# revdotcom/reverb

Measured on AMD Instinct MI355X. Metric: RTFx (audio-sec/wall-sec) Reverb-ASR attention_rescoring, higher is better.
Workload: dtype bf16

## Files before the change

### reverb_amd/csrc/fbank.hip

```cpp
#include <algorithm>
#include <cmath>
#include <vector>

#include "../../include/rvb.h"
#include "common.h"
#include "kernels.h"

namespace rvb {

static constexpr int WIN = 400, SHIFT = 160, NFFT = 512, NBIN = 257, NMEL = 80;

__device__ __forceinline__ void fbank_frame(const float (&x)[7], bool live, int lane, float* re, float* im, float* out,
                                            const FbankTables& t) {
  float sum = 0.f;
#pragma unroll
  for (int i = 0; i < 7; ++i) sum += x[i];
  const float mean = wave_sum(sum) / (float)WIN;
#pragma unroll
  for (int i = 0; i < 7; ++i) {
    const int j = lane + 64 * i;
    if (j < WIN) im[j] = x[i] - mean;
  }
  __syncthreads();
  float y[8];
#pragma unroll
  for (int i = 0; i < 8; ++i) {
    const int j = lane + 64 * i;
    float v = 0.f;
    if (j < WIN) {
      const float cur = im[j];
      const float prev = im[j > 0 ? j - 1 : 0];
      v = (cur - 0.97f * prev) * t.window[j];
    }
    y[i] = v;
  }
  __syncthreads();
#pragma unroll
  for (int i = 0; i < 8; ++i) {
    const int j = lane + 64 * i;
    re[__brev((unsigned)j) >> 23] = y[i];
    im[j] = 0.f;
  }
  __syncthreads();
#pragma unroll 1
  for (int s = 0; s < 9; ++s) {
    const int half = 1 << s;
#pragma unroll
    for (int q = 0; q < 4; ++q) {
      const int b = lane + 64 * q;
      const int j = b & (half - 1);
      const int i0 = ((b >> s) << (s + 1)) + j;
      const int i1 = i0 + half;
      const int tw = j << (8 - s);
      const float wr = t.twiddle[2 * tw], wi = t.twiddle[2 * tw + 1];
      const float ar = re[i0], ai = im[i0], br = re[i1], bi = im[i1];
      const float tr = wr * br - wi * bi;
      const float ti = wr * bi + wi * br;
      re[i0] = ar + tr; im[i0] = ai + ti;
      re[i1] = ar - tr; im[i1] = ai - ti;
    }
    __syncthreads();
  }
  float pw[5];
#pragma unroll
  for (int i = 0; i < 5; ++i) {
    const int j = lane + 64 * i;
    pw[i] = (j < NBIN) ? re[j] * re[j] + im[j] * im[j] : 0.f;
  }
  __syncthreads();
#pragma unroll
  for (int i = 0; i < 5; ++i) {
    const int j = lane + 64 * i;
    if (j < NBIN) re[j] = pw[i];
  }
  __syncthreads();
  if (live) {
#pragma unroll
    for (int i = 0; i < 2; ++i) {
      const int m = lane + 64 * i;
      if (m < NMEL) {
        const int lo = t.mel_lo[m], hi = t.mel_hi[m];
        const float* wrow = t.mel_w + (size_t)m * NBIN;
        float acc = 0.f;
        for (int b = lo; b < hi; ++b) acc += re[b] * wrow[b];
        out[m] = logf(fmaxf(acc, 1.1920928955078125e-07f));
      }
    }
  }
}

template <typename In>
__device__ __forceinline__ void fbank_load(const In* __restrict__ src, bool live, int lane, float (&x)[7]) {
#pragma unroll
  for (int i = 0; i < 7; ++i) {
    const int j = lane + 64 * i;
    x[i] = (live && j < WIN) ? (float)src[j] : 0.f;
  }
}

template <typename In>
__global__ __launch_bounds__(256) void fbank_kernel(const In* __restrict__ pcm, int64_t n_frames,
                                                    float* __restrict__ feats, FbankTables t) {
  __shared__ float s_re[4][NFFT];
  __shared__ float s_im[4][NFFT];
  const int lane = threadIdx.x & 63;
  const int w = threadIdx.x >> 6;
  const int64_t frame = (int64_t)blockIdx.x * 4 + w;
  const bool live = frame < n_frames;
  float x[7];
  fbank_load(pcm + frame * SHIFT, live, lane, x);
  fbank_frame(x, live, lane, s_re[w], s_im[w], feats + frame * NMEL, t);
}

__global__ __launch_bounds__(256) void fbank_batch_kernel(const int16_t* __restrict__ pcm, const float* __restrict__ wave,
                                                          const int64_t* __restrict__ frame0, const FbankRec* __restrict__ rec,
                                                          int n_rec, float* __restrict__ feats, FbankTables t) {
  __shared__ float s_re[4][NFFT];
  __shared__ float s_im[4][NFFT];
  const int lane = threadIdx.x & 63;
  const int w = __builtin_amdgcn_readfirstlane(threadIdx.x >> 6);
  const int64_t frame = (int64_t)blockIdx.x * 4 + w;
  const bool live = frame < frame0[n_rec];
  float x[7];
  float* out = feats;
  if (live) {
    int lo = 0, hi = n_rec;
    while (hi - lo > 1) {
      const int mid = (lo + hi) >> 1;
      if (frame0[mid] <= frame) lo = mid; else hi = mid;
    }
    const FbankRec r = rec[lo];
    const int64_t local = frame - frame0[lo];
    out = feats + (r.row0 + local) * NMEL;
    if (r.is_float) fbank_load(wave + r.src + local * SHIFT, true, lane, x);
    else fbank_load(pcm + r.src + local * SHIFT, true, lane, x);
  } else {
#pragma unroll
    for (int i = 0; i < 7; ++i) x[i] = 0.f;
  }
  fbank_frame(x, live, lane, s_re[w], s_im[w], out, t);
}

int fbank(hipStream_t s, const int16_t* pcm, int64_t n_frames, float* feats, const FbankTables& t) {
  if (n_frames <= 0) return OK;
  hipLaunchKernelGGL(fbank_kernel<int16_t>, dim3(cdiv(n_frames, 4)), dim3(256), 0, s, pcm, n_frames, feats, t);
  RVB_HIP_CHECK(hipGetLastError());
  return OK;
}

int fbank_f32(hipStream_t s, const float* wave, int64_t n_frames, float* feats, const FbankTables& t) {
  if (n_frames <= 0) return OK;
  hipLaunchKernelGGL(fbank_kernel<float>, dim3(cdiv(n_frames, 4)), dim3(256), 0, s, wave, n_frames, feats, t);
  RVB_HIP_CHECK(hipGetLastError());
  return OK;
}

int fbank_batch(hipStream_t s, const int16_t* pcm, const float* wave, const int64_t* frame0, const FbankRec* rec, int n_rec,
                int64_t total_frames, float* feats, int64_t n_rows, const FbankTables& t) {
  if (n_rows > 0) RVB_HIP_CHECK(hipMemsetAsync(feats, 0, (size_t)n_rows * NMEL * 4, s));
  if (total_frames <= 0 || n_rec <= 0) return OK;
  hipLaunchKernelGGL(fbank_batch_kernel, dim3(cdiv(total_frames, 4)), dim3(256), 0, s, pcm, wave, frame0, rec, n_rec, feats, t);
  RVB_HIP_CHECK(hipGetLastError());
  return OK;
}

template <typename In>
__global__ __launch_bounds__(256) void resample_kernel(const In* __restrict__ pcm, int64_t n_in, const float* __restrict__ ker,
                                                       int orig, int new_, int width, int K, float* __restrict__ out,
                                                       int64_t n_out) {
  const int64_t n = (int64_t)blockIdx.x * 256 + threadIdx.x;
  if (n >= n_out) return;
  const int64_t j = n / new_;
  const int p = (int)(n - j * new_);
  const int64_t base = j * orig - width;
  const float* kr = ker + (size_t)p * K;
  float acc = 0.f;
  for (int k = 0; k < K; ++k) {
    const int64_t i = base + k;
    if (i >= 0 && i < n_in) acc = fmaf(kr[k], (float)pcm[i], acc);
  }
  out[n] = acc;
}
int resample(hipStream_t s, const int16_t* pcm, int64_t n_in, const float* ker, int orig, int new_, int width, int K, float* out,
             int64_t n_out) {
  if (n_out <= 0) return OK;
  hipLaunchKernelGGL(resample_kernel<int16_t>, dim3(cdiv(n_out, 256)), dim3(256), 0, s, pcm, n_in, ker, orig, new_, width, K, out, n_out);
  RVB_HIP_CHECK(hipGetLastError());
  return OK;
}

int resample_f32(hipStream_t s, const float* pcm, int64_t n_in, const float* ker, int orig, int new_, int width, int K, float* out,
             int64_t n_out) {
  if (n_out <= 0) return OK;
  hipLaunchKernelGGL(resample_kernel<float>, dim3(cdiv(n_out, 256)), dim3(256), 0, s, pcm, n_in, ker, orig, new_, width, K, out, n_out);
  RVB_HIP_CHECK(hipGetLastError());
  return OK;
}

void resample_taps(int sample_rate, int target, std::vector<float>* ker, int* orig_out, int* new_out, int* width_out, int* K_out) {
  int a = sample_rate, b = target;
  while (b) { const int t = a % b; a = b; b = t; }
  const int orig = sample_rate / a, nw = target / a;
  const double lpw = 6.0, rolloff = 0.99;
  const double base_freq = std::min(orig, nw) * rolloff;
  const int width = (int)std::ceil(lpw * orig / base_freq);
  const int K = 2 * width + orig;
  ker->assign((size_t)nw * K, 0.f);
  const double PI = 3.14159265358979323846;
  for (int p = 0; p < nw; ++p)
    for (int k = 0; k < K; ++k) {
      double t = (-(double)p / nw + (double)(k - width) / orig) * base_freq;
      t = std::max(-lpw, std::min(lpw, t));
      const double c = std::cos(t * PI / lpw / 2.0);
      const double window = c * c;
      t *= PI;
      const double sinc = t == 0.0 ? 1.0 : std::sin(t) / t;
      (*ker)[(size_t)p * K + k] = (float)(sinc * window * (base_freq / orig));
    }
  *orig_out = orig; *new_out = nw; *width_out = width; *K_out = K;
}

struct FbankAny { int win, shift, nmel; };
__global__ __launch_bounds__(256) void fbank_any_kernel(const float* __restrict__ wave, int64_t n_frames, float* __restrict__ feats,
                                                        FbankTables t, FbankAny g) {
  __shared__ float s_re[4][NFFT];
  __shared__ float s_im[4][NFFT];
  const int lane = threadIdx.x & 63;
  const int w = threadIdx.x >> 6;
  const int64_t frame = (int64_t)blockIdx.x * 4 + w;
  const bool live = frame < n_frames;
  float* re = s_re[w];
  float* im = s_im[w];
  float x[8];
  float sum = 0.f;
  const float* src = wave + frame * g.shift;
#pragma unroll
  for (int i = 0; i < 8; ++i) {
    const int j = lane + 64 * i;
    x[i] = (live && j < g.win) ? src[j] : 0.f;
    sum += x[i];
  }
  const float mean = wave_sum(sum) / (float)g.win;
#pragma unroll
  for (int i = 0; i < 8; ++i) {
    const int j = lane + 64 * i;
    if (j < g.win) im[j] = x[i] - mean;
  }
  __syncthreads();
  float y[8];
#pragma unroll
  for (int i = 0; i < 8; ++i) {
    const int j = lane + 64 * i;
    float v = 0.f;
    if (j < g.win) v = (im[j] - 0.97f * im[j > 0 ? j - 1 : 0]) * t.window[j];
    y[i] = v;
  }
  __syncthreads();
#pragma unroll
  for (int i = 0; i < 8; ++i) {
    const int j = lane + 64 * i;
    re[__brev((unsigned)j) >> 23] = y[i];
    im[j] = 0.f;
  }
  __syncthreads();
#pragma unroll 1
  for (int s = 0; s < 9; ++s) {
    const int half = 1 << s;
#pragma unroll
    for (int q = 0; q < 4; ++q) {
      const int b = lane + 64 * q;
      const int j = b & (half - 1);
      const int i0 = ((b >> s) << (s + 1)) + j;
      const int i1 = i0 + half;
      const int tw = j << (8 - s);
      const float wr = t.twiddle[2 * tw], wi = t.twiddle[2 * tw + 1];
      const float ar = re[i0], ai = im[i0], br = re[i1], bi = im[i1];
      const float tr = wr * br - wi * bi;
      const float ti = wr * bi + wi * br;
      re[i0] = ar + tr; im[i0] = ai + ti;
      re[i1] = ar - tr; im[i1] = ai - ti;
    }
    __syncthreads();
  }
  float pw[5];
#pragma unroll
  for (int i = 0; i < 5; ++i) {
    const int j = lane + 64 * i;
    pw[i] = (j < NBIN) ? re[j] * re[j] + im[j] * im[j] : 0.f;
  }
  __syncthreads();
#pragma unroll
  for (int i = 0; i < 5; ++i) {
    const int j = lane + 64 * i;
    if (j < NBIN) re[j] = pw[i];
  }
  __syncthreads();
  if (live) {
#pragma unroll
    for (int i = 0; i < 2; ++i) {
      const int m = lane + 64 * i;
      if (m < g.nmel) {
        const int lo = t.mel_lo[m], hi = t.mel_hi[m];
        const float* wrow = t.mel_w + (size_t)m * NBIN;
        float acc = 0.f;
        for (int b = lo; b < hi; ++b) acc += re[b] * wrow[b];
        feats[frame * g.nmel + m] = logf(fmaxf(acc, 1.1920928955078125e-07f));
      }
    }
  }
}

void fbank_host_tables(int win, int nmel, std::vector<float>* window, std::vector<float>* tw, std::vector<float>* melw,
                       std::vector<int32_t>* lo, std::vector<int32_t>* hi) {
  const double PI = 3.14159265358979323846;
  window->resize(win); tw->resize(2 * 256); melw->assign((size_t)nmel * NBIN, 0.f);
  lo->assign(nmel, NBIN); hi->assign(nmel, 0);
  for (int i = 0; i < win; ++i) (*window)[i] = (float)std::pow(0.5 - 0.5 * std::cos(2.0 * PI * i / (win - 1)), 0.85);
  for (int k = 0; k < 256; ++k) { (*tw)[2 * k] = (float)std::cos(2.0 * PI * k / NFFT); (*tw)[2 * k + 1] = (float)(-std::sin(2.0 * PI * k / NFFT)); }
  auto mel = [](double f) { return 1127.0 * std::log(1.0 + f / 700.0); };
  const double mlo = mel(20.0), mhi = mel(8000.0), delta = (mhi - mlo) / (nmel + 1);
  for (int m = 0; m < nmel; ++m) {
    const double left = mlo + m * delta, center = left + delta, right = center + delta;
    for (int b = 0; b < NFFT / 2; ++b) {
      const double mf = mel(16000.0 / NFFT * b);
      const double up = (mf - left) / (center - left), down = (right - mf) / (right - center);
      const double wgt = std::max(0.0, std::min(up, down));
      if (wgt > 0.0) {
        (*melw)[(size_t)m * NBIN + b] = (float)wgt;
        (*lo)[m] = std::min((*lo)[m], b); (*hi)[m] = std::max((*hi)[m], b + 1);
      }
    }
    if ((*hi)[m] == 0) (*lo)[m] = 0;
  }
}

int fbank_any(hipStream_t s, const float* wave, int64_t n_frames, float* feats, const FbankTables& t, int win, int shift, int nmel) {
  if (n_frames <= 0) return OK;
  const FbankAny g{win, shift, nmel};
  hipLaunchKernelGGL(fbank_any_kernel, dim3(cdiv(n_frames, 4)), dim3(256), 0, s, wave, n_frames, feats, t, g);
  RVB_HIP_CHECK(hipGetLastError());
  return OK;
}

__global__ __launch_bounds__(256) void round_i16_kernel(const float* __restrict__ x, int64_t n, int16_t* __restrict__ out) {
  const int64_t i = (int64_t)blockIdx.x * 256 + threadIdx.x;
  if (i < n) out[i] = (int16_t)__builtin_rintf(fminf(fmaxf(x[i], -32768.f), 32767.f));
}
int round_to_i16(hipStream_t s, const float* x, int64_t n, int16_t* out) {
  if (n <= 0) return OK;
  hipLaunchKernelGGL(round_i16_kernel, dim3(cdiv(n, 256)), dim3(256), 0, s, x, n, out);
  RVB_HIP_CHECK(hipGetLastError());
  return OK;
}

}

extern "C" int rvb_compute_feats(int device, const float* wave, int64_t n_samples, int num_mel_bins, double frame_length_ms,
                                 double frame_shift_ms, float* feats_out, int64_t* n_frames) {
  using namespace rvb;
  if (!n_frames || (!wave && n_samples > 0) || n_samples < 0) { set_error("rvb_compute_feats: bad argument"); return E_ARG; }
  const int win = (int)(16000.0 * frame_length_ms * 0.001), shift = (int)(16000.0 * frame_shift_ms * 0.001);
  if (win <= 256 || win > 512 || shift < 1 || num_mel_bins < 1 || num_mel_bins > 128) {
    set_error("rvb_compute_feats: supported are frame_length 16.1 .. 32 ms (a 512-point FFT at 16 kHz), frame_shift >= 1 sample, 1 .. 128 mel bins");
    return E_UNSUPPORTED;
  }
  const int64_t nf = n_samples < win ? 0 : 1 + (n_samples - win) / shift;
  *n_frames = nf;
  if (!feats_out || nf == 0) return OK;
  int ndev = 0;
  if (hipGetDeviceCount(&ndev) != hipSuccess || ndev <= device || device < 0) { set_error("rvb_compute_feats: no HIP device (this library has no CPU fallback)"); return E_HIP; }
  RVB_HIP_CHECK(hipSetDevice(device));
  std::vector<float> window, tw, melw;
  std::vector<int32_t> lo, hi;
  fbank_host_tables(win, num_mel_bins, &window, &tw, &melw, &lo, &hi);
  void *dwave = nullptr, *dwin = nullptr, *dtw = nullptr, *dmel = nullptr, *dlo = nullptr, *dhi = nullptr, *dout = nullptr;
  auto up = [](void** d, const void* h, size_t bytes) { return hipMalloc(d, bytes) == hipSuccess && hipMemcpy(*d, h, bytes, hipMemcpyHostToDevice) == hipSuccess; };
  int rc = OK;
  if (!up(&dwave, wave, (size_t)n_samples * 4) || !up(&dwin, window.data(), window.size() * 4) || !up(&dtw, tw.data(), tw.size() * 4) ||
      !up(&dmel, melw.data(), melw.size() * 4) || !up(&dlo, lo.data(), lo.size() * 4) || !up(&dhi, hi.data(), hi.size() * 4) ||
      hipMalloc(&dout, (size_t)nf * num_mel_bins * 4) != hipSuccess) {
    set_error("rvb_compute_feats: device allocation / upload failed"); rc = E_NOMEM;
  }
  if (rc == OK) {
    const FbankTables t{(const float*)dwin, (const float*)dtw, (const float*)dmel, (const int*)dlo, (const int*)dhi};
    rc = fbank_any(nullptr, (const float*)dwave, nf, (float*)dout, t, win, shift, num_mel_bins);
    if (rc == OK && hipDeviceSynchronize() != hipSuccess) { set_error("rvb_compute_feats: kernel failed"); rc = E_HIP; }
    if (rc == OK && hipMemcpy(feats_out, dout, (size_t)nf * num_mel_bins * 4, hipMemcpyDeviceToHost) != hipSuccess) { set_error("rvb_compute_feats: download failed"); rc = E_HIP; }
  }
  for (void* q : {dwave, dwin, dtw, dmel, dlo, dhi, dout}) if (q) (void)hipFree(q);
  return rc;
}
```

Before: 27840.

## Rewrite fbank as persistent register-radix-8 FFT with staged mel weights

```diff
diff --git a/reverb_amd/csrc/fbank.hip b/reverb_amd/csrc/fbank.hip
--- a/reverb_amd/csrc/fbank.hip
+++ b/reverb_amd/csrc/fbank.hip
@@ -9,148 +9,289 @@
 namespace rvb {
 
 static constexpr int WIN = 400, SHIFT = 160, NFFT = 512, NBIN = 257, NMEL = 80;
-
-__device__ __forceinline__ void fbank_frame(const float (&x)[7], bool live, int lane, float* re, float* im, float* out,
-                                            const FbankTables& t) {
+static constexpr int FB_GROUP = 4;
+static constexpr int FB_ITEMS = FB_GROUP * NMEL / 64;
+static constexpr int FB_PW_STRIDE = 264;
+static constexpr int FB_MELW_CAP = 1024;
+static constexpr int FB_BLOCKS_PER_CU = 4;
+
+__device__ __forceinline__ void wave_lds_fence() {
+  __builtin_amdgcn_fence(__ATOMIC_RELEASE, "wavefront");
+  __builtin_amdgcn_wave_barrier();
+  __builtin_amdgcn_fence(__ATOMIC_ACQUIRE, "wavefront");
+}
+
+typedef float fb_f2 __attribute__((ext_vector_type(2)));
+typedef float fb_f4 __attribute__((ext_vector_type(4)));
+typedef __attribute__((address_space(3))) fb_f2 fb_lds_f2;
+typedef __attribute__((address_space(3))) fb_f4 fb_lds_f4;
+
+struct FbankShared {
+  fb_f2 xch[4][NFFT];
+  float pw[4][FB_GROUP][FB_PW_STRIDE];
+  float melw[FB_MELW_CAP];
+  int mel_off[NMEL + 1];
+  int mel_wd[NMEL];
+  int mel_lo[NMEL];
+  float win[448];
+  int64_t row[4][FB_GROUP];
+};
+
+struct FbankLane {
+  float wr[3][7], wi[3][7];
+  int x1w, x1r, x2w, x2r;
+};
+
+__device__ __forceinline__ void fbank_lane(int lane, const FbankTables& t, FbankLane* c) {
+  const int hi1 = (int)(__brev((unsigned)(lane & 7)) >> 29), mid1 = (int)(__brev((unsigned)(lane >> 3)) >> 29);
+  const int lo2 = ((lane >> 5) << 2) | (lane & 3), hi2 = (lane >> 2) & 7;
+  const int mid3 = lane >> 3, lo3 = lane & 7;
+  c->x1w = (mid1 << 6) | (hi1 << 1);
+  c->x1r = ((lo2 >> 2) << 5) | (((lo2 >> 1) & 1) << 4) | (hi2 << 1) | (lo2 & 1);
+  c->x2w = ((lo2 & 3) << 1) | ((hi2 & 1) << 3) | ((lo2 >> 2) << 4) | ((hi2 >> 1) << 7);
+  c->x2r = (mid3 & 1) | ((lo3 & 3) << 1) | (((mid3 >> 1) & 1) << 3) | ((lo3 >> 2) << 4) | (((mid3 >> 1) & 1) << 5) | ((mid3 >> 2) << 6);
+  const int lam[3] = {0, lo2, lane};
+#pragma unroll
+  for (int p = 0; p < 3; ++p)
+#pragma unroll
+    for (int tt = 0; tt < 3; ++tt)
+#pragma unroll
+      for (int j = 0; j < (1 << tt); ++j) {
+        const int stride = p == 0 ? 1 : p == 1 ? 8 : 64;
+        const int tw = (lam[p] + stride * j) << (8 - 3 * p - tt);
+        c->wr[p][(1 << tt) - 1 + j] = t.twiddle[2 * tw];
+        c->wi[p][(1 << tt) - 1 + j] = t.twiddle[2 * tw + 1];
+      }
+}
+
+__device__ __forceinline__ bool fbank_stage_mel(FbankShared& sh, const FbankTables& t) {
+  const int tid = threadIdx.x;
+  if (tid < NMEL) {
+    sh.mel_lo[tid] = t.mel_lo[tid];
+    sh.mel_wd[tid] = max(t.mel_hi[tid] - t.mel_lo[tid], 0);
+  }
+  for (int j = tid; j < 448; j += 256) sh.win[j] = j < WIN ? t.window[j] : 0.f;
+  __syncthreads();
+  if (tid <= NMEL) {
+    int o = 0;
+    for (int m = 0; m < tid; ++m) o += sh.mel_wd[m];
+    sh.mel_off[tid] = o;
+  }
+  __syncthreads();
+  const bool staged = sh.mel_off[NMEL] <= FB_MELW_CAP;
+  if (staged) {
+    for (int m = tid >> 6; m < NMEL; m += 4) {
+      const int lo = sh.mel_lo[m], wd = sh.mel_wd[m], off = sh.mel_off[m];
+      for (int i = tid & 63; i < wd; i += 64) sh.melw[off + i] = t.mel_w[(size_t)m * NBIN + lo + i];
+    }
+  }
+  __syncthreads();
+  return staged;
+}
+
+__device__ __forceinline__ void fbank_pass(float (&re)[8], float (&im)[8], const float (&wr)[7], const float (&wi)[7]) {
+#pragma clang fp contract(off)
+#pragma unroll
+  for (int t = 0; t < 3; ++t) {
+#pragma unroll
+    for (int k0 = 0; k0 < 8; ++k0) {
+      if (k0 & (1 << t)) continue;
+      const int k1 = k0 + (1 << t), n = (1 << t) - 1 + (k0 & ((1 << t) - 1));
+      const float ar = re[k0], ai = im[k0], br = re[k1], bi = im[k1];
+      const float tr = __builtin_fmaf(wr[n], br, -(wi[n] * bi));
+      const float ti = __builtin_fmaf(wi[n], br, wr[n] * bi);
+      re[k0] = ar + tr; im[k0] = ai + ti;
+      re[k1] = ar - tr; im[k1] = ai - ti;
+    }
+  }
+}
+
+__device__ __forceinline__ void fbank_frame(const float (&x)[7], int lane, fb_f2* xch, float* pw, const float* win, const FbankLane& c) {
+#pragma clang fp contract(off)
+  float* stage = reinterpret_cast<float*>(xch);
   float sum = 0.f;
 #pragma unroll
   for (int i = 0; i < 7; ++i) sum += x[i];
   const float mean = wave_sum(sum) / (float)WIN;
+  float d[7];
 #pragma unroll
   for (int i = 0; i < 7; ++i) {
     const int j = lane + 64 * i;
-    if (j < WIN) im[j] = x[i] - mean;
-  }
-  __syncthreads();
+    d[i] = x[i] - mean;
+    if (j < WIN) stage[j] = d[i];
+  }
+  wave_lds_fence();
   float y[8];
 #pragma unroll
-  for (int i = 0; i < 8; ++i) {
+  for (int i = 0; i < 7; ++i) {
     const int j = lane + 64 * i;
     float v = 0.f;
     if (j < WIN) {
-      const float cur = im[j];
-      const float prev = im[j > 0 ? j - 1 : 0];
-      v = (cur - 0.97f * prev) * t.window[j];
+      const float prev = stage[j > 0 ? j - 1 : 0];
+      v = __builtin_fmaf(-0.97f, prev, d[i]) * win[j];
     }
     y[i] = v;
   }
-  __syncthreads();
-#pragma unroll
-  for (int i = 0; i < 8; ++i) {
-    const int j = lane + 64 * i;
-    re[__brev((unsigned)j) >> 23] = y[i];
-    im[j] = 0.f;
-  }
-  __syncthreads();
+  y[7] = 0.f;
+  wave_lds_fence();
+  float re[8], im[8];
+#pragma unroll
+  for (int k = 0; k < 8; ++k) {
+    re[k] = y[((k & 1) << 2) | (k & 2) | (k >> 2)];
+    im[k] = 0.f;
+  }
+  fbank_pass(re, im, c.wr[0], c.wi[0]);
+  volatile fb_lds_f4* xch4 = (volatile fb_lds_f4*)xch;
+  const volatile fb_lds_f2* xch2 = (const volatile fb_lds_f2*)xch;
+#pragma unroll
+  for (int p = 0; p < 4; ++p) xch4[(c.x1w | (p << 4)) >> 1] = fb_f4{re[2 * p], im[2 * p], re[2 * p + 1], im[2 * p + 1]};
+  wave_lds_fence();
+#pragma unroll
+  for (int k = 0; k < 8; ++k) {
+    const fb_f2 v = xch2[c.x1r | (k << 6)];
+    re[k] = v.x; im[k] = v.y;
+  }
+  fbank_pass(re, im, c.wr[1], c.wi[1]);
+  wave_lds_fence();
+#pragma unroll
+  for (int p = 0; p < 4; ++p)
+    xch4[((c.x2w ^ ((p & 1) * 0x28)) | ((p >> 1) << 6)) >> 1] = fb_f4{re[2 * p], im[2 * p], re[2 * p + 1], im[2 * p + 1]};
+  wave_lds_fence();
+#pragma unroll
+  for (int k = 0; k < 8; ++k) {
+    const fb_f2 v = xch2[(c.x2r ^ ((k & 1) << 3)) | ((k >> 1) << 7)];
+    re[k] = v.x; im[k] = v.y;
+  }
+  fbank_pass(re, im, c.wr[2], c.wi[2]);
+  wave_lds_fence();
+#pragma unroll
+  for (int k = 0; k < 4; ++k) pw[lane + 64 * k] = __builtin_fmaf(re[k], re[k], im[k] * im[k]);
+  const float nyq = re[4] * re[4] + im[4] * im[4];
+  if (lane == 0) pw[256] = nyq;
+}
+
+__device__ __forceinline__ void fbank_mel(int lane, const float* pw, const int64_t* row, const FbankShared& sh, bool staged,
+                                          const FbankTables& t, float* __restrict__ feats) {
+#pragma clang fp contract(off)
+#pragma unroll
+  for (int i = 0; i < FB_ITEMS; ++i) {
+    const int it = lane + 64 * i, m = it >> 2, q = it & 3;
+    const int64_t r = row[q];
+    if (r < 0) continue;
+    const int lo = sh.mel_lo[m], wd = sh.mel_wd[m];
+    const float* p = pw + q * FB_PW_STRIDE + lo;
+    float acc = 0.f;
+    if (staged) {
+      const float* w = sh.melw + sh.mel_off[m];
+      for (int b = 0; b < wd; ++b) acc = __builtin_fmaf(p[b], w[b], acc);
+    } else {
+      const float* w = t.mel_w + (size_t)m * NBIN + lo;
+      for (int b = 0; b < wd; ++b) acc = __builtin_fmaf(p[b], w[b], acc);
+    }
+    feats[r * NMEL + m] = logf(fmaxf(acc, 1.1920928955078125e-07f));
+  }
+}
+
+template <typename In>
+__device__ __forceinline__ void fbank_load(const In* __restrict__ src, int lane, float (&x)[7]) {
+#pragma unroll
+  for (int i = 0; i < 7; ++i) {
+    const int j = lane + 64 * i;
+    x[i] = j < WIN ? (float)src[j] : 0.f;
+  }
+}
+
+template <typename In>
+__global__ __launch_bounds__(256) __attribute__((amdgpu_waves_per_eu(4, 4))) void fbank_kernel(const In* __restrict__ pcm, int64_t n_frames,
+                                                    float* __restrict__ feats, FbankTables t) {
+  __shared__ FbankShared sh;
+  const int lane = threadIdx.x & 63;
+  const int w = __builtin_amdgcn_readfirstlane(threadIdx.x >> 6);
+  const bool staged = fbank_stage_mel(sh, t);
+  FbankLane c;
+  fbank_lane(lane, t, &c);
+  const int64_t n_groups = (n_frames + FB_GROUP - 1) / FB_GROUP;
+  for (int64_t g = (int64_t)blockIdx.x * 4 + w; g < n_groups; g += (int64_t)gridDim.x * 4) {
 #pragma unroll 1
-  for (int s = 0; s < 9; ++s) {
-    const int half = 1 << s;
-#pragma unroll
-    for (int q = 0; q < 4; ++q) {
-      const int b = lane + 64 * q;
-      const int j = b & (half - 1);
-      const int i0 = ((b >> s) << (s + 1)) + j;
-      const int i1 = i0 + half;
-      const int tw = j << (8 - s);
-      const float wr = t.twiddle[2 * tw], wi = t.twiddle[2 * tw + 1];
-      const float ar = re[i0], ai = im[i0], br = re[i1], bi = im[i1];
-      const float tr = wr * br - wi * bi;
-      const float ti = wr * bi + wi * br;
-      re[i0] = ar + tr; im[i0] = ai + ti;
-      re[i1] = ar - tr; im[i1] = ai - ti;
-    }
-    __syncthreads();
-  }
-  float pw[5];
-#pragma unroll
-  for (int i = 0; i < 5; ++i) {
-    const int j = lane + 64 * i;
-    pw[i] = (j < NBIN) ? re[j] * re[j] + im[j] * im[j] : 0.f;
-  }
-  __syncthreads();
-#pragma unroll
-  for (int i = 0; i < 5; ++i) {
-    const int j = lane + 64 * i;
-    if (j < NBIN) re[j] = pw[i];
-  }
-  __syncthreads();
-  if (live) {
-#pragma unroll
-    for (int i = 0; i < 2; ++i) {
-      const int m = lane + 64 * i;
-      if (m < NMEL) {
-        const int lo = t.mel_lo[m], hi = t.mel_hi[m];
-        const float* wrow = t.mel_w + (size_t)m * NBIN;
-        float acc = 0.f;
-        for (int b = lo; b < hi; ++b) acc += re[b] * wrow[b];
-        out[m] = logf(fmaxf(acc, 1.1920928955078125e-07f));
+    for (int q = 0; q < FB_GROUP; ++q) {
+      const int64_t frame = g * FB_GROUP + q;
+      const bool live = frame < n_frames;
+      sh.row[w][q] = live ? frame : -1;
+      if (live) {
+        float x[7];
+        fbank_load(pcm + frame * SHIFT, lane, x);
+        fbank_frame(x, lane, sh.xch[w], sh.pw[w][q], sh.win, c);
       }
     }
-  }
-}
-
-template <typename In>
-__device__ __forceinline__ void fbank_load(const In* __restrict__ src, bool live, int lane, float (&x)[7]) {
-#pragma unroll
-  for (int i = 0; i < 7; ++i) {
-    const int j = lane + 64 * i;
-    x[i] = (live && j < WIN) ? (float)src[j] : 0.f;
-  }
-}
-
-template <typename In>
-__global__ __launch_bounds__(256) void fbank_kernel(const In* __restrict__ pcm, int64_t n_frames,
-                                                    float* __restrict__ feats, FbankTables t) {
-  __shared__ float s_re[4][NFFT];
-  __shared__ float s_im[4][NFFT];
-  const int lane = threadIdx.x & 63;
-  const int w = threadIdx.x >> 6;
-  const int64_t frame = (int64_t)blockIdx.x * 4 + w;
-  const bool live = frame < n_frames;
-  float x[7];
-  fbank_load(pcm + frame * SHIFT, live, lane, x);
-  fbank_frame(x, live, lane, s_re[w], s_im[w], feats + frame * NMEL, t);
-}
-
-__global__ __launch_bounds__(256) void fbank_batch_kernel(const int16_t* __restrict__ pcm, const float* __restrict__ wave,
+    wave_lds_fence();
+    fbank_mel(lane, &sh.pw[w][0][0], sh.row[w], sh, staged, t, feats);
+    wave_lds_fence();
+  }
+}
+
+__global__ __launch_bounds__(256) __attribute__((amdgpu_waves_per_eu(4, 4))) void fbank_batch_kernel(const int16_t* __restrict__ pcm, const float* __restrict__ wave,
                                                           const int64_t* __restrict__ frame0, const FbankRec* __restrict__ rec,
                                                           int n_rec, float* __restrict__ feats, FbankTables t) {
-  __shared__ float s_re[4][NFFT];
-  __shared__ float s_im[4][NFFT];
+  __shared__ FbankShared sh;
   const int lane = threadIdx.x & 63;
   const int w = __builtin_amdgcn_readfirstlane(threadIdx.x >> 6);
-  const int64_t frame = (int64_t)blockIdx.x * 4 + w;
-  const bool live = frame < frame0[n_rec];
-  float x[7];
-  float* out = feats;
-  if (live) {
-    int lo = 0, hi = n_rec;
-    while (hi - lo > 1) {
-      const int mid = (lo + hi) >> 1;
-      if (frame0[mid] <= frame) lo = mid; else hi = mid;
-    }
-    const FbankRec r = rec[lo];
-    const int64_t local = frame - frame0[lo];
-    out = feats + (r.row0 + local) * NMEL;
-    if (r.is_float) fbank_load(wave + r.src + local * SHIFT, true, lane, x);
-    else fbank_load(pcm + r.src + local * SHIFT, true, lane, x);
-  } else {
-#pragma unroll
-    for (int i = 0; i < 7; ++i) x[i] = 0.f;
-  }
-  fbank_frame(x, live, lane, s_re[w], s_im[w], out, t);
+  const bool staged = fbank_stage_mel(sh, t);
+  FbankLane c;
+  fbank_lane(lane, t, &c);
+  const int64_t n_frames = frame0[n_rec];
+  const int64_t n_groups = (n_frames + FB_GROUP - 1) / FB_GROUP;
+  for (int64_t g = (int64_t)blockIdx.x * 4 + w; g < n_groups; g += (int64_t)gridDim.x * 4) {
+#pragma unroll 1
+    for (int q = 0; q < FB_GROUP; ++q) {
+      const int64_t frame = g * FB_GROUP + q;
+      const bool live = frame < n_frames;
+      int64_t row = -1;
+      if (live) {
+        int lo = 0, hi = n_rec;
+        while (hi - lo > 1) {
+          const int mid = (lo + hi) >> 1;
+          if (frame0[mid] <= frame) lo = mid; else hi = mid;
+        }
+        const FbankRec r = rec[lo];
+        const int64_t local = frame - frame0[lo];
+        row = r.row0 + local;
+        float x[7];
+        if (r.is_float) fbank_load(wave + r.src + local * SHIFT, lane, x);
+        else fbank_load(pcm + r.src + local * SHIFT, lane, x);
+        fbank_frame(x, lane, sh.xch[w], sh.pw[w][q], sh.win, c);
+      }
+      sh.row[w][q] = row;
+    }
+    wave_lds_fence();
+    fbank_mel(lane, &sh.pw[w][0][0], sh.row[w], sh, staged, t, feats);
+    wave_lds_fence();
+  }
+}
+
+static int fbank_blocks(hipStream_t s, int64_t n_frames, int* blocks) {
+  int dev = 0, cus = 0;
+  if (s) RVB_HIP_CHECK(hipStreamGetDevice(s, &dev));
+  else RVB_HIP_CHECK(hipGetDevice(&dev));
+  RVB_HIP_CHECK(hipDeviceGetAttribute(&cus, hipDeviceAttributeMultiprocessorCount, dev));
+  const int64_t want = (n_frames + 4 * FB_GROUP - 1) / (4 * FB_GROUP);
+  *blocks = (int)std::max<int64_t>(1, std::min<int64_t>(want, (int64_t)std::max(cus, 1) * FB_BLOCKS_PER_CU));
+  return OK;
 }
 
 int fbank(hipStream_t s, const int16_t* pcm, int64_t n_frames, float* feats, const FbankTables& t) {
   if (n_frames <= 0) return OK;
-  hipLaunchKernelGGL(fbank_kernel<int16_t>, dim3(cdiv(n_frames, 4)), dim3(256), 0, s, pcm, n_frames, feats, t);
+  int blocks = 0;
+  RVB_TRY(fbank_blocks(s, n_frames, &blocks));
+  hipLaunchKernelGGL(fbank_kernel<int16_t>, dim3(blocks), dim3(256), 0, s, pcm, n_frames, feats, t);
   RVB_HIP_CHECK(hipGetLastError());
   return OK;
 }
 
 int fbank_f32(hipStream_t s, const float* wave, int64_t n_frames, float* feats, const FbankTables& t) {
   if (n_frames <= 0) return OK;
-  hipLaunchKernelGGL(fbank_kernel<float>, dim3(cdiv(n_frames, 4)), dim3(256), 0, s, wave, n_frames, feats, t);
+  int blocks = 0;
+  RVB_TRY(fbank_blocks(s, n_frames, &blocks));
+  hipLaunchKernelGGL(fbank_kernel<float>, dim3(blocks), dim3(256), 0, s, wave, n_frames, feats, t);
   RVB_HIP_CHECK(hipGetLastError());
   return OK;
 }
@@ -159,7 +300,9 @@
                 int64_t total_frames, float* feats, int64_t n_rows, const FbankTables& t) {
   if (n_rows > 0) RVB_HIP_CHECK(hipMemsetAsync(feats, 0, (size_t)n_rows * NMEL * 4, s));
   if (total_frames <= 0 || n_rec <= 0) return OK;
-  hipLaunchKernelGGL(fbank_batch_kernel, dim3(cdiv(total_frames, 4)), dim3(256), 0, s, pcm, wave, frame0, rec, n_rec, feats, t);
+  int blocks = 0;
+  RVB_TRY(fbank_blocks(s, total_frames, &blocks));
+  hipLaunchKernelGGL(fbank_batch_kernel, dim3(blocks), dim3(256), 0, s, pcm, wave, frame0, rec, n_rec, feats, t);
   RVB_HIP_CHECK(hipGetLastError());
   return OK;
 }
```

New measurement: 27830. Within noise of the previous version (-0.0%).
